# mrluin/TextualDegRemoval

Measured on AMD Instinct MI355X. Metric: train images/sec (512x512, bs=4/GPU), higher is better.
Workload: dtype f32 (3xbf16-split MFMA: 24-bit operand significands on the full fp32 exponent range, fp32 accumulate; unscaled gradients, no loss scale, no step-skip guard; tensors fp32 -- the MASA-encoder ResidualBlock activations / gradients as three bf16 planes whose sum IS the fp32 value, bit for bit)

## Files before the change

### textualdegremoval_amd/csrc/tdr_common.h

```cpp
#pragma once
#include <hip/hip_runtime.h>
#include <stdint.h>
#include <stdio.h>
#include <string.h>

#define TDR_OK 0
#define TDR_ERR_ARG (-1)
#define TDR_ERR_HIP (-2)
#define TDR_ERR_UNSUPPORTED (-3)

void tdr_set_error(const char* fmt, ...);

#define TDR_REQUIRE(cond, ...)                     \
    do {                                           \
        if (!(cond)) {                             \
            tdr_set_error(__VA_ARGS__);            \
            return TDR_ERR_ARG;                    \
        }                                          \
    } while (0)

#define TDR_LAUNCH_CHECK(name)                                                         \
    do {                                                                               \
        hipError_t e__ = hipGetLastError();                                            \
        if (e__ != hipSuccess) {                                                       \
            tdr_set_error("%s: launch failed: %s", name, hipGetErrorString(e__));      \
            return TDR_ERR_HIP;                                                        \
        }                                                                              \
    } while (0)

struct TdrConvDesc;
int tdr_conv_forward_bx3(const TdrConvDesc* d, void* stream);

static inline int tdr_cdiv(long a, long b) { return (int)((a + b - 1) / b); }

#include <stdlib.h>
#ifdef TDR_TUNING_KNOBS
static inline const char* tdr_tune_env(const char* name) { return getenv(name); }
#else
static inline const char* tdr_tune_env(const char*) { return nullptr; }
#endif

__device__ __forceinline__ int tdr_xcd_logical_block() {
    const int T = gridDim.x, b = blockIdx.x;
    const int q = T >> 3, r = T & 7, xcd = b & 7, slot = b >> 3;
    return (xcd < r ? xcd * (q + 1) : r * (q + 1) + (xcd - r) * q) + slot;
}

typedef __attribute__((ext_vector_type(16))) float f32x16;
typedef __attribute__((ext_vector_type(4))) float f32x4;

__device__ __forceinline__ float wave_sum(float v) {
#pragma unroll
    for (int o = 32; o > 0; o >>= 1) v += __shfl_xor(v, o, 64);
    return v;
}
template <int CTRL>
__device__ __forceinline__ float dpp_perm(float v) {
    return __builtin_bit_cast(float, __builtin_amdgcn_update_dpp(0, __builtin_bit_cast(int, v), CTRL, 0xf, 0xf, true));
}
__device__ __forceinline__ float wave_sum_dpp(float v) {
    v += dpp_perm<0xB1>(v);
    v += dpp_perm<0x4E>(v);
    v += dpp_perm<0x141>(v);
    v += dpp_perm<0x140>(v);
    const int b = __builtin_bit_cast(int, v);
    return (__builtin_bit_cast(float, __builtin_amdgcn_readlane(b, 0)) + __builtin_bit_cast(float, __builtin_amdgcn_readlane(b, 16))) +
           (__builtin_bit_cast(float, __builtin_amdgcn_readlane(b, 32)) + __builtin_bit_cast(float, __builtin_amdgcn_readlane(b, 48)));
}
__device__ __forceinline__ float wave_max(float v) {
#pragma unroll
    for (int o = 32; o > 0; o >>= 1) v = fmaxf(v, __shfl_xor(v, o, 64));
    return v;
}

typedef float tdr_f32x2 __attribute__((ext_vector_type(2)));
typedef _Float16 tdr_f16x2 __attribute__((ext_vector_type(2)));
template <bool PIN = true>
__device__ __forceinline__ void tdr_split2_f16(float x0, float x1, unsigned& h, unsigned& m) {
    if constexpr (PIN) asm volatile("" : "+v"(x0), "+v"(x1));
    const tdr_f32x2 xv = {x0, x1};
    h = __builtin_bit_cast(unsigned, __builtin_convertvector(xv, tdr_f16x2));
    const float neg1 = -1.0f;
    asm("v_fma_mixlo_f16 %0, %1, %2, %3 op_sel:[0,0,0] op_sel_hi:[1,0,0]" : "=v"(m) : "v"(h), "v"(neg1), "v"(x0));
    asm("v_fma_mixhi_f16 %0, %1, %2, %3 op_sel:[1,0,0] op_sel_hi:[1,0,0]" : "+v"(m) : "v"(h), "v"(neg1), "v"(x1));
}

typedef __bf16 tdr_bf16x2 __attribute__((ext_vector_type(2)));
template <bool PIN = true>
__device__ __forceinline__ void tdr_split3_bf16(float x0, float x1, unsigned& h, unsigned& m, unsigned& l) {
    if constexpr (PIN) asm volatile("" : "+v"(x0), "+v"(x1));
    const tdr_f32x2 xv = {x0, x1};
    h = __builtin_bit_cast(unsigned, __builtin_convertvector(xv, tdr_bf16x2));
    const float r0 = x0 - __builtin_bit_cast(float, h << 16), r1 = x1 - __builtin_bit_cast(float, h & 0xffff0000u);
    const tdr_f32x2 rv = {r0, r1};
    m = __builtin_bit_cast(unsigned, __builtin_convertvector(rv, tdr_bf16x2));
    const tdr_f32x2 sv = {r0 - __builtin_bit_cast(float, m << 16), r1 - __builtin_bit_cast(float, m & 0xffff0000u)};
    l = __builtin_bit_cast(unsigned, __builtin_convertvector(sv, tdr_bf16x2));
}
```

### textualdegremoval_amd/csrc/tdr_dwsg.hip

```cpp
#include <stdlib.h>
#include "tdr_common.h"
#include "tdr_erf.h"
#include "tdr_dw_stencil.h"
#include "../../include/tdr.h"

namespace {

enum { MODE_FWD = 0, MODE_DU = 1, MODE_DT = 2 };
enum { GATE_MUL = 0, GATE_GELU = 1, GATE_NONE = 2, GATE_SUM = 3 };

__device__ __forceinline__ float gelu_erf(float x) { return 0.5f * x * (1.0f + erf_1ulp(x * 0.70710678118654752f)); }
__device__ __forceinline__ void gelu_erf_both(float x, float& g, float& dg) {
    const float h = 0.5f * (1.0f + erf_1ulp(x * 0.70710678118654752f));
    g = x * h;
    dg = h + x * 0.3989422804014327f * __expf(-0.5f * x * x);
}

struct DwArgs {
    const float* a;
    const float* dg;
    const float* w;
    const float* b;
    float* out;
    float* part;
// ... 272 lines not shown
                for (int kx = 0; kx < 3; ++kx)
#pragma unroll
                    for (int e = 0; e < 4; ++e) {
                        o1[e] += w1[ky * 3 + kx] * t1[ky].v[e + kx];
                        o2[e] += w2[ky * 3 + kx] * t2[ky].v[e + kx];
                    }
            if (GATE == GATE_MUL && in_img) gv += dgb;
            float d1[4], d2[4];
#pragma unroll
            for (int e = 0; e < 4; ++e) {
                if (GATE == GATE_GELU) {
                    float gl, gd;
                    gelu_erf_both(o1[e], gl, gd);
                    d1[e] = gv[e] * o2[e] * gd;
                    d2[e] = gv[e] * gl;
                } else {
                    d1[e] = gv[e] * o2[e];
                    d2[e] = gv[e] * o1[e];
                }
                if (!in_img) { d1[e] = 0.f; d2[e] = 0.f; }
            }
            float l1 = __shfl_up(d1[3], 1, 64), r1 = __shfl_down(d1[0], 1, 64);
            float l2 = __shfl_up(d2[3], 1, 64), r2 = __shfl_down(d2[0], 1, 64);
            if (!left_lane) { l1 = 0.f; l2 = 0.f; }
            if (!right_lane) { r1 = 0.f; r2 = 0.f; }
            if (TPRW > 64) {
                const int wv = tid >> 6, par = i & 1;
                if (lane == 0) { edge[par][wv][0] = d1[0]; edge[par][wv][1] = d2[0]; }
                if (lane == 63) { edge[par][wv][2] = d1[3]; edge[par][wv][3] = d2[3]; }
                __syncthreads();
                if (lane == 0 && cg != 0) { l1 = edge[par][wv - 1][2]; l2 = edge[par][wv - 1][3]; }
                if (lane == 63 && cg != TPRW - 1) { r1 = edge[par][wv + 1][0]; r2 = edge[par][wv + 1][1]; }
            }
            e1[2].v[0] = l1; e1[2].v[5] = r1; e2[2].v[0] = l2; e2[2].v[5] = r2;
#pragma unroll
            for (int e = 0; e < 4; ++e) { e1[2].v[e + 1] = d1[e]; e2[2].v[e + 1] = d2[e]; }
        }
        if (i >= 1 && i <= a.rpt && in_img) {
#pragma unroll
            for (int ky = 0; ky < 3; ++ky)
#pragma unroll
                for (int kx = 0; kx < 3; ++kx)
#pragma unroll
                    for (int e = 0; e < 4; ++e) {
                        acc[ky * 3 + kx] += e1[2].v[e + 1] * t1[ky].v[e + kx];
                        acc[10 + ky * 3 + kx] += e2[2].v[e + 1] * t2[ky].v[e + kx];
                    }
            acc[9] += (e1[2].v[1] + e1[2].v[2]) + (e1[2].v[3] + e1[2].v[4]);
            acc[19] += (e2[2].v[1] + e2[2].v[2]) + (e2[2].v[3] + e2[2].v[4]);
        }
        if (i >= 2) {
            const int yo = y - 1;
            float o1[4] = {0.f, 0.f, 0.f, 0.f}, o2[4] = {0.f, 0.f, 0.f, 0.f};
#pragma unroll
            for (int ky = 0; ky < 3; ++ky)
#pragma unroll
                for (int kx = 0; kx < 3; ++kx)
#pragma unroll
                    for (int e = 0; e < 4; ++e) {
                        o1[e] += w1[8 - (ky * 3 + kx)] * e1[ky].v[e + kx];
                        o2[e] += w2[8 - (ky * 3 + kx)] * e2[ky].v[e + kx];
                    }
            if (active && yo < H) {
                const f32x4 v1 = {o1[0], o1[1], o1[2], o1[3]}, v2 = {o2[0], o2[1], o2[2], o2[3]};
                *reinterpret_cast<f32x4*>(a.out + ((long)n * 2 * C + pl1) * HW + (long)yo * W + x0) = v1;
                *reinterpret_cast<f32x4*>(a.out + ((long)n * 2 * C + pl2) * HW + (long)yo * W + x0) = v2;
            }
        }
        t1[0] = t1[1]; t1[1] = t1[2];
        t2[0] = t2[1]; t2[1] = t2[2];
        e1[0] = e1[1]; e1[1] = e1[2];
        e2[0] = e2[1]; e2[1] = e2[2];
    }
#pragma unroll
    for (int i = 0; i < 20; ++i) {
        const float s = wave_sum(acc[i]);
        if (lane == 0) red[tid >> 6][i] = s;
    }
    __syncthreads();
    if (tid < 20)
        a.part[(((long)n * C + c) * gridDim.x + blockIdx.x) * 20 + tid] = (red[0][tid] + red[1][tid]) + (red[2][tid] + red[3][tid]);
}

__global__ void dw_param_finish_kernel(const float* __restrict__ part, int N, int C, int nb, float* __restrict__ dw,
                                       float* __restrict__ db, int sum_pairs) {
    const int c = blockIdx.x, tid = threadIdx.x;
    if (tid >= 20) return;
    float sacc = 0.f;
    for (int m = 0; m < N; ++m)
        for (int g = 0; g < nb; ++g) sacc += part[(((long)m * C + c) * nb + g) * 20 + tid];
    const int kk = tid % 10;
    if (sum_pairs) {
        if (kk < 9) dw[(2 * c + (tid >= 10)) * 9 + kk] = sacc;
        else if (db && tid == 9) db[c] = sacc;
        return;
    }
    const int ch = tid < 10 ? c : c + C;
    if (kk < 9) dw[ch * 9 + kk] = sacc;
    else if (db) db[ch] = sacc;
}

__global__ void dw_param_finish_multi_kernel(const long long* __restrict__ tab) {
    const long long* row = tab + 6L * blockIdx.y;
    const int N = (int)row[3], C = (int)row[4], nb = (int)row[5];
    if ((int)blockIdx.x >= C) return;
    const float* part = reinterpret_cast<const float*>(row[0]);
    float* dw = reinterpret_cast<float*>(row[1]);
    float* db = reinterpret_cast<float*>(row[2]);
    const int c = blockIdx.x, tid = threadIdx.x;
    if (tid >= 20) return;
    float sacc = 0.f;
    for (int m = 0; m < N; ++m)
        for (int g = 0; g < nb; ++g) sacc += part[(((long)m * C + c) * nb + g) * 20 + tid];
    const int kk = tid % 10;
    const int ch = tid < 10 ? c : c + C;
    if (kk < 9) dw[ch * 9 + kk] = sacc;
    else db[ch] = sacc;
}

DwGeom dw_geom_fused(int H, int W) {
    DwGeom g = dw_geom(H, W);
    const int spb = 256 >> g.tprw_log2;
    static const int cap = tdr_tune_env("TDR_DWF_RPT") ? atoi(tdr_tune_env("TDR_DWF_RPT")) : 16;
    int rpt = tdr_cdiv(H, spb);
    if (rpt > cap) rpt = cap;
    if (rpt < 1) rpt = 1;
    g.rpt = rpt;
    g.nby = tdr_cdiv(H, spb * rpt);
    g.nb = g.ncb * g.nby;
    return g;
}

bool dw_two_pass() {
    const char* e = getenv("TDR_DWSG_TWO_PASS");
    return e && e[0] == '1';
}

template <int GATE>
int dw_bwd_fused(const float* t, const float* dg, const float* dg_bias, float dg_bias_mul, const float* w, const float* b, int N,
                 int C, int H, int W, float* dt, float* dw, float* db, float* ws, hipStream_t st, const float* act = nullptr,
                 long dg_ns = 0, long act_ns = 0, const float* dgB = nullptr, const float* actB = nullptr) {
    const DwGeom q = dw_geom_fused(H, W);
    DwArgs a{t, dg, w, b, dt, ws, C, H, W, q.tprw_log2, q.rpt, q.ncb, 1.0f, nullptr, nullptr, dg_bias, dg_bias_mul, act,
             {0, dg_ns, act_ns}, nullptr, 0, dgB, dg_ns, actB, act_ns};
    hipLaunchKernelGGL((dwsg_bwd_fused_kernel<GATE>), dim3(q.nb, C, N), dim3(256), 0, st, a);
    if (dw)
        hipLaunchKernelGGL(dw_param_finish_kernel, dim3(C), dim3(32), 0, st, ws, N, C, q.nb, dw, db, GATE == GATE_SUM ? 1 : 0);
    return 0;
}

}

extern "C" int64_t tdr_dwsg_ws_floats(int N, int C, int H, int W) {
    const DwGeom g = dw_geom(H, W);
    return (int64_t)N * C * g.nb * 20 + 4 + (int64_t)N * 2 * C * H * W;
}

extern "C" int tdr_dwsg_fwd(const float* t, const float* w, const float* b, int N, int C, int H, int W, float* g, float* pooled,
                            float* ws, void* stream) {
    TDR_REQUIRE(t && w && b && g && pooled && ws, "tdr_dwsg_fwd: null pointer");
    TDR_REQUIRE(W % 4 == 0, "tdr_dwsg_fwd: W must be a multiple of 4 (got %d)", W);
    hipStream_t st = (hipStream_t)stream;
    const DwGeom q = dw_geom(H, W);
    const float inv_hw = 1.0f / (float)((long)H * W);
    if (q.nb == 1) {
        DwArgs a{t, nullptr, w, b, g, pooled, C, H, W, q.tprw_log2, q.rpt, q.ncb, inv_hw};
        hipLaunchKernelGGL((dwsg_stencil_kernel<MODE_FWD, GATE_MUL>), dim3(q.nb, C, N), dim3(256), 0, st, a);
        TDR_LAUNCH_CHECK("dwsg_fwd");
        return TDR_OK;
    }
    DwArgs a{t, nullptr, w, b, g, ws, C, H, W, q.tprw_log2, q.rpt, q.ncb, 1.0f};
    hipLaunchKernelGGL((dwsg_stencil_kernel<MODE_FWD, GATE_MUL>), dim3(q.nb, C, N), dim3(256), 0, st, a);
    hipLaunchKernelGGL(dw_pool_finish_kernel, dim3(tdr_cdiv(N * C, 256)), dim3(256), 0, st, ws, N * C, q.nb, inv_hw, pooled);
    TDR_LAUNCH_CHECK("dwsg_fwd");
    return TDR_OK;
}

extern "C" int tdr_dwsg_bwd_parts_supported(int W) { return (W <= 1024 && !dw_two_pass()) ? 1 : 0; }

extern "C" int tdr_dw_param_finish(const float* ws, int N, int C, int H, int W, float* dw, float* db, void* stream) {
    TDR_REQUIRE(ws && dw && db && N > 0 && C > 0, "tdr_dw_param_finish: bad argument");
    const DwGeom q = dw_geom_fused(H, W);
    hipLaunchKernelGGL(dw_param_finish_kernel, dim3(C), dim3(32), 0, (hipStream_t)stream, const_cast<float*>(ws), N, C, q.nb, dw, db, 0);
    TDR_LAUNCH_CHECK("dw_param_finish_kernel");
    return TDR_OK;
}

extern "C" int tdr_dw_param_finish_nb(int H, int W) { return dw_geom_fused(H, W).nb; }

extern "C" int tdr_dw_param_finish_multi(const void* table, int nprob, int max_C, void* stream) {
    TDR_REQUIRE(table && nprob > 0 && max_C > 0, "tdr_dw_param_finish_multi: bad argument");
    hipLaunchKernelGGL(dw_param_finish_multi_kernel, dim3(max_C, nprob), dim3(32), 0, (hipStream_t)stream, static_cast<const long long*>(table));
    TDR_LAUNCH_CHECK("dw_param_finish_multi_kernel");
    return TDR_OK;
}

extern "C" int tdr_dwsg_bwd(const float* dg, const float* t, const float* w, const float* b, int N, int C, int H, int W,
                            float* dt, float* dw, float* db, float* ws, void* stream) {
    return tdr_dwsg_bwd_biased(dg, nullptr, 0.f, t, w, b, N, C, H, W, dt, dw, db, ws, stream);
}

extern "C" int tdr_dwsg_bwd_biased(const float* dg, const float* dg_bias, float dg_bias_mul, const float* t, const float* w,
                                   const float* b, int N, int C, int H, int W, float* dt, float* dw, float* db, float* ws,
                                   void* stream) {
    TDR_REQUIRE(dg && t && w && b && dt && ws, "tdr_dwsg_bwd: null pointer");
    TDR_REQUIRE((dw != nullptr) == (db != nullptr), "tdr_dwsg_bwd: dw and db are given together or not at all");
    TDR_REQUIRE(dw || tdr_dwsg_bwd_parts_supported(W), "tdr_dwsg_bwd: dw = db = NULL (partials left to the caller) needs the one-pass backward");
    TDR_REQUIRE(W % 4 == 0, "tdr_dwsg_bwd: W must be a multiple of 4 (got %d)", W);
    hipStream_t st = (hipStream_t)stream;
    if (W <= 1024 && !dw_two_pass()) {
        dw_bwd_fused<GATE_MUL>(t, dg, dg_bias, dg_bias_mul, w, b, N, C, H, W, dt, dw, db, ws, st);
        TDR_LAUNCH_CHECK("dwsg_bwd_fused");
        return TDR_OK;
    }
    const DwGeom q = dw_geom(H, W);
    float* part = ws;
    float* du = ws + (int64_t)N * C * q.nb * 20;
    du += (4 - (reinterpret_cast<uintptr_t>(du) / 4) % 4) % 4;
    DwArgs a1{t, dg, w, b, du, part, C, H, W, q.tprw_log2, q.rpt, q.ncb, 1.0f, nullptr, nullptr, dg_bias, dg_bias_mul};
    hipLaunchKernelGGL((dwsg_stencil_kernel<MODE_DU, GATE_MUL>), dim3(q.nb, C, N), dim3(256), 0, st, a1);
    DwArgs a2{du, nullptr, w, b, dt, part, C, H, W, q.tprw_log2, q.rpt, q.ncb, 1.0f, dw, db};
    hipLaunchKernelGGL((dwsg_stencil_kernel<MODE_DT, GATE_MUL>), dim3(q.nb, C, N), dim3(256), 0, st, a2);
    TDR_LAUNCH_CHECK("dwsg_bwd");
    return TDR_OK;
}

extern "C" int tdr_dwgelu_fwd(const float* t, const float* w, const float* b, int N, int C, int H, int W, float* g,
                              void* stream) {
// ... 127 lines not shown
```

### textualdegremoval_amd/csrc/tdr_pointwise.hip

```cpp
#include "tdr_common.h"
#include "../../include/tdr.h"

namespace {

template <int SLICES, int CPT>
__global__ __launch_bounds__(64 * SLICES) void ln_fwd_kernel(const float* __restrict__ x, long x_ns,
                                                            const float* __restrict__ w, const float* __restrict__ b,
                                                            float eps, int center, int C, int HW,
                                                            float* __restrict__ y, float* __restrict__ mu,
                                                            float* __restrict__ rstd) {
    __shared__ float red[SLICES][64];
    const int lane = threadIdx.x & 63, slice = threadIdx.x >> 6;
    const int px = blockIdx.x * 64 + lane, n = blockIdx.y;
    const bool pok = px < HW;
    const float* xn = x + (long)n * x_ns + (pok ? px : HW - 1);
    float v[CPT];
    float s = 0.f;
#pragma unroll
    for (int i = 0; i < CPT; ++i) v[i] = xn[(long)min(slice + SLICES * i, C - 1) * HW];
#pragma unroll
    for (int i = 0; i < CPT; ++i) {
        v[i] = (pok && slice + SLICES * i < C) ? v[i] : 0.f;
        s += v[i];
    }
// ... 120 lines not shown
    for (int c = slice; c < C; c += 16) yn[(long)c * HW] = (xn[(long)c * HW] - mo) * rs * w[c] + (b ? b[c] : 0.f);
    if (slice == 0) {
        mu[(long)n * HW + px] = mean;
        rstd[(long)n * HW + px] = rs;
    }
}

template <int SLICES, int CPT>
__global__ __launch_bounds__(64 * SLICES) void ln_bwd_kernel(
    const float* __restrict__ go, const float* __restrict__ x, long x_ns, const float* __restrict__ mu,
    const float* __restrict__ rstd, const float* __restrict__ w, const float* __restrict__ add, long add_ns, int add_C,
    int center, int N, int C, int HW, float* __restrict__ gx, float* __restrict__ part ) {
    __shared__ float red[2][SLICES][64];
    const int lane = threadIdx.x & 63, slice = __builtin_amdgcn_readfirstlane(threadIdx.x >> 6);
    const int tiles = (HW + 63) / 64;
    float aw[CPT], ab[CPT];
#pragma unroll
    for (int i = 0; i < CPT; ++i) { aw[i] = 0.f; ab[i] = 0.f; }
    const unsigned uHW = (unsigned)HW;
    for (int t = blockIdx.x; t < N * tiles; t += gridDim.x) {
        const int n = t / tiles, px = (t % tiles) * 64 + lane;
        const bool pok = px < HW;
        const unsigned pxc = pok ? px : HW - 1;
        const float m = mu[(long)n * HW + pxc], rs = pok ? rstd[(long)n * HW + pxc] : 0.f;
        const float* xb = x + (long)n * x_ns;
        const float* gb_ = go + (long)n * C * HW;
        float* ob = gx + (long)n * C * HW;
        float xv[CPT], g0[CPT];
#pragma unroll
        for (int i = 0; i < CPT; ++i) {
            const unsigned c = min(slice + SLICES * i, C - 1);
            xv[i] = xb[c * uHW + pxc];
            g0[i] = gb_[c * uHW + pxc];
        }
        const float off = center ? 0.f : m * rs;
        float s1 = 0.f, s2 = 0.f;
#pragma unroll
        for (int i = 0; i < CPT; ++i) {
            const int c = slice + SLICES * i;
            const bool ok = pok && c < C;
            const float gg = ok ? g0[i] : 0.f;
            const float yh = ok ? (xv[i] - m) * rs : 0.f;
            const float yu = ok ? yh + off : 0.f;
            const float gv = gg * w[min(c, C - 1)];
            xv[i] = yh; g0[i] = gv;
            s1 += gv;
            s2 += gv * yu;
            aw[i] += gg * yu;
            ab[i] += gg;
        }
        red[0][slice][lane] = s1;
        red[1][slice][lane] = s2;
        __syncthreads();
        float S1 = 0.f, S2 = 0.f;
#pragma unroll
        for (int k = 0; k < SLICES; ++k) { S1 += red[0][k][lane]; S2 += red[1][k][lane]; }
        __syncthreads();
        const float mg = center ? S1 / (float)C : 0.f, mgy = S2 / (float)C;
        float av[CPT];
        if (add) {
            const float* ab_ = add + (long)n * add_ns;
#pragma unroll
            for (int i = 0; i < CPT; ++i) av[i] = ab_[(unsigned)min(slice + SLICES * i, add_C - 1) * uHW + pxc];
        }
#pragma unroll
        for (int i = 0; i < CPT; ++i) {
            const int c = slice + SLICES * i;
            float v = rs * (g0[i] - xv[i] * mgy - mg);
            if (add && c < add_C) v += av[i];
            if (pok && c < C) ob[(unsigned)c * uHW + pxc] = v;
        }
    }
#pragma unroll
    for (int i = 0; i < CPT; ++i) {
        const int c = slice + SLICES * i;
        const float sw = wave_sum(aw[i]), sb = wave_sum(ab[i]);
        if (lane == 0 && c < C) {
            part[((long)blockIdx.x * 2 + 0) * C + c] = sw;
            part[((long)blockIdx.x * 2 + 1) * C + c] = sb;
        }
    }
}

template <bool PART>
__global__ __launch_bounds__(1024) void ln_bwd_generic_kernel(
    const float* __restrict__ go, const float* __restrict__ x, long x_ns, const float* __restrict__ mu,
    const float* __restrict__ rstd, const float* __restrict__ w, const float* __restrict__ add, long add_ns, int add_C,
    int center, int C, int HW, float* __restrict__ gx, float* __restrict__ part) {
    __shared__ float red[2][16][64];
    const int lane = threadIdx.x & 63, slice = threadIdx.x >> 6;
    const int px = blockIdx.x * 64 + lane, n = blockIdx.y;
    const bool pok = px < HW;
    const unsigned pxc = pok ? px : HW - 1, uHW = (unsigned)HW;
    const float m = mu[(long)n * HW + pxc], rs = rstd[(long)n * HW + pxc];
    const float* xb = x + (long)n * x_ns;
    const float* gb_ = go + (long)n * C * HW;
    const float off = center ? 0.f : m * rs;
    float s1 = 0.f, s2 = 0.f;
#pragma unroll 4
    for (int c = slice; c < C; c += 16) {
        const float g = gb_[(unsigned)c * uHW + pxc] * w[c];
        const float yh = (xb[(unsigned)c * uHW + pxc] - m) * rs;
        s1 += g; s2 += g * (yh + off);
    }
    red[0][slice][lane] = s1; red[1][slice][lane] = s2;
    __syncthreads();
    float S1 = 0.f, S2 = 0.f;
#pragma unroll
    for (int k = 0; k < 16; ++k) { S1 += red[0][k][lane]; S2 += red[1][k][lane]; }
    const float mg = center ? S1 / (float)C : 0.f, mgy = S2 / (float)C;
    const float* ab_ = add ? add + (long)n * add_ns : xb;
    float* ob = gx + (long)n * C * HW;
    for (int c0 = slice; c0 < C; c0 += 64) {
        float g0[4], xv[4], av[4];
#pragma unroll
        for (int k = 0; k < 4; ++k) {
            const int c = min(c0 + 16 * k, C - 1);
            g0[k] = gb_[(unsigned)c * uHW + pxc];
            xv[k] = xb[(unsigned)c * uHW + pxc];
            av[k] = ab_[(unsigned)min(c, add ? add_C - 1 : C - 1) * uHW + pxc];
        }
#pragma unroll
        for (int k = 0; k < 4; ++k) {
            const int c = c0 + 16 * k;
            if (c < C) {
                const float g = g0[k] * w[c];
                const float yh = (xv[k] - m) * rs;
                float v = rs * (g - yh * mgy - mg);
                if (add && c < add_C) v += av[k];
                if (pok) ob[(unsigned)c * uHW + pxc] = v;
                if (PART) {
                    const float sw = wave_sum(pok ? g0[k] * (yh + off) : 0.f), sb = wave_sum(pok ? g0[k] : 0.f);
                    if (lane == 0) {
                        float* pb = part + ((long)(blockIdx.y * gridDim.x + blockIdx.x) * 2) * C;
                        pb[c] = sw;
                        pb[C + c] = sb;
                    }
                }
            }
        }
    }
}

template <int CPT>
__global__ __launch_bounds__(1024) void ln_bwd_cached_kernel(
    const float* __restrict__ go, const float* __restrict__ x, long x_ns, const float* __restrict__ mu,
    const float* __restrict__ rstd, const float* __restrict__ w, const float* __restrict__ add, long add_ns, int add_C,
    int center, int C, int HW, float* __restrict__ gx, float* __restrict__ part) {
    __shared__ float red[2][16][64];
    const int lane = threadIdx.x & 63, slice = __builtin_amdgcn_readfirstlane(threadIdx.x >> 6);
    const int px = blockIdx.x * 64 + lane, n = blockIdx.y;
    const bool pok = px < HW;
    const unsigned pxc = pok ? px : HW - 1;
    const float* xb = x + (long)n * x_ns;
    const float* gb_ = go + (long)n * C * HW;
    float g0[CPT], xv[CPT];
#pragma unroll
    for (int i = 0; i < CPT; ++i) {
        const long row = (long)min(slice + 16 * i, C - 1) * HW;
        g0[i] = (gb_ + row)[pxc];
        xv[i] = (xb + row)[pxc];
    }
    const float m = mu[(long)n * HW + pxc], rs = rstd[(long)n * HW + pxc];
    const float off = center ? 0.f : m * rs;
    float s1 = 0.f, s2 = 0.f;
#pragma unroll
    for (int i = 0; i < CPT; ++i) {
        const int c = slice + 16 * i;
        const float wc = c < C ? w[min(c, C - 1)] : 0.f;
        g0[i] = c < C ? g0[i] : 0.f;
        xv[i] = (xv[i] - m) * rs;
        const float g = g0[i] * wc;
        s1 += g; s2 += g * (xv[i] + off);
    }
    red[0][slice][lane] = s1; red[1][slice][lane] = s2;
    __syncthreads();
    float S1 = 0.f, S2 = 0.f;
#pragma unroll
    for (int k = 0; k < 16; ++k) { S1 += red[0][k][lane]; S2 += red[1][k][lane]; }
    const float mg = center ? S1 / (float)C : 0.f, mgy = S2 / (float)C;
    const float* ab_ = add ? add + (long)n * add_ns : xb;
    float* ob = gx + (long)n * C * HW;
    float* pb = part + ((long)(blockIdx.y * gridDim.x + blockIdx.x) * 2) * C;
#pragma unroll
    for (int i = 0; i < CPT; ++i) {
        const int c = slice + 16 * i, cc = min(c, C - 1);
        const long row = (long)cc * HW;
        float v = rs * (g0[i] * w[cc] - xv[i] * mgy - mg);
        const float av = (ab_ + (long)min(cc, add ? add_C - 1 : C - 1) * HW)[pxc];
        if (add && c < add_C) v += av;
        const float sw = wave_sum_dpp(pok ? g0[i] * (xv[i] + off) : 0.f), sb = wave_sum_dpp(pok ? g0[i] : 0.f);
        if (c < C) {
            if (pok) (ob + row)[pxc] = v;
            if (lane == 0) { pb[c] = sw; pb[C + c] = sb; }
        }
    }
}

__global__ __launch_bounds__(256) void ln_param_grad_kernel(const float* __restrict__ go, const float* __restrict__ x,
                                                           long x_ns, const float* __restrict__ mu,
                                                           const float* __restrict__ rstd, int center, int N, int C,
                                                           int HW, float* __restrict__ part) {
    __shared__ float red[2][4];
    const int c = blockIdx.x, split = blockIdx.y, nsplit = gridDim.y;
    const long total = (long)N * HW;
    float sw = 0.f, sb = 0.f;
    for (long i = (long)split * 256 + threadIdx.x; i < total; i += (long)nsplit * 256) {
        const int n = (int)(i / HW), px = (int)(i % HW);
        const float g0 = go[((long)n * C + c) * HW + px];
        const float yh = (x[(long)n * x_ns + (long)c * HW + px] - (center ? mu[i] : 0.f)) * rstd[i];
        sw += g0 * yh; sb += g0;
    }
    sw = wave_sum(sw); sb = wave_sum(sb);
    if ((threadIdx.x & 63) == 0) { red[0][threadIdx.x >> 6] = sw; red[1][threadIdx.x >> 6] = sb; }
    __syncthreads();
    if (threadIdx.x == 0) {
        part[((long)split * 2 + 0) * C + c] = red[0][0] + red[0][1] + red[0][2] + red[0][3];
        part[((long)split * 2 + 1) * C + c] = red[1][0] + red[1][1] + red[1][2] + red[1][3];
    }
}

template <int KL>
__global__ __launch_bounds__(64 * KL) void pair_sum_partials_kernel(const float* __restrict__ part, int nparts, int C,
                                                                    float* __restrict__ o0, float* __restrict__ o1) {
    __shared__ float red[KL][64];
    const int lane = threadIdx.x & 63, kl = threadIdx.x >> 6;
    const int e = blockIdx.x * 64 + lane;
    const int ec = e < C ? e : C - 1;
    const float* p = part + (long)blockIdx.y * C + ec;
    const long stride = 2L * C;
    float s0 = 0.f, s1 = 0.f;
    int k = kl;
    for (; k + KL < nparts; k += 2 * KL) { s0 += p[(long)k * stride]; s1 += p[(long)(k + KL) * stride]; }
    if (k < nparts) s0 += p[(long)k * stride];
    red[kl][lane] = s0 + s1;
    __syncthreads();
    if (kl == 0 && e < C) {
        float t = 0.f;
#pragma unroll
        for (int q = 0; q < KL; ++q) t += red[q][lane];
        (blockIdx.y ? o1 : o0)[e] = t;
    }
}

template <int KL>
__global__ __launch_bounds__(64 * KL) void pair_sum_partials_multi_kernel(const long long* __restrict__ tab) {
    __shared__ float red[KL][64];
    const long long* row = tab + 5L * blockIdx.z;
    const int nparts = (int)row[3], C = (int)row[4];
    if ((int)blockIdx.x * 64 >= C) return;
    const float* part = reinterpret_cast<const float*>(row[0]);
    float* o = reinterpret_cast<float*>(blockIdx.y ? row[2] : row[1]);
    const int lane = threadIdx.x & 63, kl = threadIdx.x >> 6;
    const int e = blockIdx.x * 64 + lane;
    const int ec = e < C ? e : C - 1;
    const float* p = part + (long)blockIdx.y * C + ec;
    const long stride = 2L * C;
    float s0 = 0.f, s1 = 0.f;
    int k = kl;
    for (; k + KL < nparts; k += 2 * KL) { s0 += p[(long)k * stride]; s1 += p[(long)(k + KL) * stride]; }
    if (k < nparts) s0 += p[(long)k * stride];
    red[kl][lane] = s0 + s1;
    __syncthreads();
    if (kl == 0 && e < C) {
        float t = 0.f;
#pragma unroll
        for (int q = 0; q < KL; ++q) t += red[q][lane];
        o[e] = t;
    }
}

constexpr int LN_BWD_GRID = 1024;
static const int ln_bwd_grid = tdr_tune_env("TDR_LN_BWD_GRID") ? atoi(tdr_tune_env("TDR_LN_BWD_GRID")) : 256;
constexpr int LN_GEN_SPLITS = 16;

__global__ __launch_bounds__(256) void sca_fwd_kernel(const float* __restrict__ pooled, const float* __restrict__ wsca,
                                                     const float* __restrict__ bsca, int C, float* __restrict__ s) {
    const int co = blockIdx.x * 4 + (threadIdx.x >> 6), n = blockIdx.y, lane = threadIdx.x & 63;
    if (co >= C) return;
    float a = 0.f;
    for (int ci = lane; ci < C; ci += 64) a += wsca[(long)co * C + ci] * pooled[(long)n * C + ci];
    a = wave_sum(a);
    if (lane == 0) s[(long)n * C + co] = a + bsca[co];
}

__global__ __launch_bounds__(256) void sca_bwd_rows_kernel(const float* __restrict__ G3, const float* __restrict__ S3,
                                                          const float* __restrict__ w3, const float* __restrict__ b3,
                                                          const float* __restrict__ beta, const float* __restrict__ s,
                                                          int N, int C, float* __restrict__ dw3, float* __restrict__ db3,
                                                          float* __restrict__ dbeta) {
    __shared__ float red[4];
    const int co = blockIdx.x;
    const float bt = beta[co];
    float acc = 0.f;
    for (int ci = threadIdx.x; ci < C; ci += 256) {
        float sg = 0.f;
        for (int n = 0; n < N; ++n) sg += s[(long)n * C + ci] * G3[((long)n * C + co) * C + ci];
        dw3[(long)co * C + ci] = bt * sg;
        acc += w3[(long)co * C + ci] * sg;
    }
    acc = wave_sum(acc);
    if ((threadIdx.x & 63) == 0) red[threadIdx.x >> 6] = acc;
    __syncthreads();
    if (threadIdx.x == 0) {
        const float tot = (red[0] + red[1]) + (red[2] + red[3]);
        db3[co] = bt * S3[co];
        dbeta[co] = tot + b3[co] * S3[co];
    }
}

__global__ __launch_bounds__(1024) void sca_bwd_ds_kernel(const float* __restrict__ G3, const float* __restrict__ w3,
                                                         const float* __restrict__ beta, int N, int C, float* __restrict__ ds) {
    __shared__ float red[16][64];
    const int lane = threadIdx.x & 63, sl = threadIdx.x >> 6;
    const int ci = blockIdx.x * 64 + lane, n = blockIdx.y;
    const int cic = min(ci, C - 1);
    float a = 0.f;
    for (int co = sl; co < C; co += 16) a += beta[co] * w3[(long)co * C + cic] * G3[((long)n * C + co) * C + cic];
    red[sl][lane] = a;
    __syncthreads();
    if (sl == 0 && ci < C) {
        float t = 0.f;
#pragma unroll
        for (int q = 0; q < 16; ++q) t += red[q][lane];
        ds[(long)n * C + ci] = t;
    }
}

__global__ void sca_bwd_dw_kernel(const float* __restrict__ ds, const float* __restrict__ pooled, int N, int C,
                                  float* __restrict__ dwsca) {
    const int cj = blockIdx.x * blockDim.x + threadIdx.x, ci = blockIdx.y;
    if (cj >= C) return;
    float a = 0.f;
    for (int n = 0; n < N; ++n) a += ds[(long)n * C + ci] * pooled[(long)n * C + cj];
    dwsca[(long)ci * C + cj] = a;
}

__global__ __launch_bounds__(1024) void sca_bwd_tail_kernel(const float* __restrict__ ds, const float* __restrict__ wsca,
                                                           int N, int C, float* __restrict__ dbsca,
                                                           float* __restrict__ dpooled) {
    __shared__ float red[16][64];
    const int lane = threadIdx.x & 63, sl = threadIdx.x >> 6;
    const int cj = blockIdx.x * 64 + lane, n = blockIdx.y;
    const int cjc = min(cj, C - 1);
    float a = 0.f;
    for (int ci = sl; ci < C; ci += 16) a += wsca[(long)ci * C + cjc] * ds[(long)n * C + ci];
    red[sl][lane] = a;
    __syncthreads();
    if (sl == 0 && cj < C) {
        float t = 0.f;
#pragma unroll
        for (int q = 0; q < 16; ++q) t += red[q][lane];
        dpooled[(long)n * C + cj] = t;
        if (n == 0) {
            float sb = 0.f;
            for (int m = 0; m < N; ++m) sb += ds[(long)m * C + cj];
            dbsca[cj] = sb;
// ... 288 lines not shown
    for (int k = 0; k < PSNR_BLOCKS; ++k) s += part[n * PSNR_BLOCKS + k];
    return s / (double)cnt;
}
__global__ __launch_bounds__(256) void psnr_grad_kernel(const float* __restrict__ p, const float* __restrict__ t, long CHW, long HW,
                                                       int toY, int N, float wscale, const TdrStepGuard* __restrict__ guard,
                                                       const double* __restrict__ part, float* __restrict__ dpred) {
    const int n = blockIdx.y;
    const long base = (long)n * CHW, cnt = toY ? HW : CHW;
    float gscale = wscale;
    if (guard) gscale *= guard->scale;
    const float f = (float)((double)gscale / (double)N / (psnr_image_mse(part, n, cnt) + 1e-8) * 2.0 / (double)cnt);
    for (long i = blockIdx.x * 256L + threadIdx.x; i < cnt; i += (long)gridDim.x * 256) {
        const float d = psnr_diff(p, t, base, HW, i, toY);
        if (!toY) {
            dpred[base + i] = f * d;
        } else {
            dpred[base + i] = f * d * (65.481f / 255.f);
            dpred[base + HW + i] = f * d * (128.553f / 255.f);
            dpred[base + 2 * HW + i] = f * d * (24.966f / 255.f);
        }
    }
}
__global__ void psnr_finish_kernel(const double* __restrict__ part, int N, long cnt, double wscale, float* __restrict__ loss) {
    double s = 0.0;
    for (int n = threadIdx.x; n < N; n += 64) s += log(psnr_image_mse(part, n, cnt) + 1e-8);
#pragma unroll
    for (int o = 32; o > 0; o >>= 1) s += __shfl_xor(s, o, 64);
    if (threadIdx.x == 0) loss[0] = (float)(s / (double)N * wscale);
}

inline int grid1d(long total, int cap = 8192) {
    long b = (total + 255) / 256;
    return (int)(b < cap ? (b < 1 ? 1 : b) : cap);
}

}

extern "C" int tdr_layernorm2d_fwd(const float* x, int64_t x_ns, const float* w, const float* b, float eps, int center,
                                   int N, int C, int HW, float* y, float* mu, float* rstd, void* stream) {
    TDR_REQUIRE(x && w && y && mu && rstd, "tdr_layernorm2d_fwd: null pointer");
    TDR_REQUIRE(N > 0 && C > 0 && HW > 0, "tdr_layernorm2d_fwd: bad shape");
    hipStream_t st = (hipStream_t)stream;
    dim3 grid(tdr_cdiv(HW, 64), N);
#define LN_FWD(S, P) hipLaunchKernelGGL((ln_fwd_kernel<S, P>), grid, dim3(64 * S), 0, st, x, (long)x_ns, w, b, eps, center, C, HW, y, mu, rstd)
    if (C <= 32) LN_FWD(4, 8);
    else if (C <= 64) LN_FWD(4, 16);
    else if (C <= 128) LN_FWD(4, 32);
    else if (C <= 256) LN_FWD(8, 32);
    else if (C <= 512) LN_FWD(16, 32);
    else if (C <= 64 * 24 && (long)grid.x * N < 512) {
        dim3 g16(tdr_cdiv(HW, 16), N);
        if (C <= 64 * 12) hipLaunchKernelGGL(ln_fwd_narrow_kernel<12>, g16, dim3(1024), 0, st, x, (long)x_ns, w, b, eps, center, C, HW, y, mu, rstd);
        else hipLaunchKernelGGL(ln_fwd_narrow_kernel<24>, g16, dim3(1024), 0, st, x, (long)x_ns, w, b, eps, center, C, HW, y, mu, rstd);
    }
    else hipLaunchKernelGGL(ln_fwd_generic_kernel, grid, dim3(1024), 0, st, x, (long)x_ns, w, b, eps, center, C, HW, y, mu, rstd);
#undef LN_FWD
    TDR_LAUNCH_CHECK("ln_fwd");
    return TDR_OK;
}

extern "C" int64_t tdr_ln_ws_floats(int N, int C, int HW) {
    (void)N; (void)HW;
    return (int64_t)LN_BWD_GRID * 2 * C;
}

extern "C" int tdr_layernorm2d_bwd(const float* go, const float* x, int64_t x_ns, const float* mu, const float* rstd,
                                   const float* w, const float* add, int64_t add_ns, int add_C, int center, int N, int C,
                                   int HW, float* gx, float* gw, float* gb, float* ws, void* stream) {
    TDR_REQUIRE(go && x && mu && rstd && w && gx && gw && gb && ws, "tdr_layernorm2d_bwd: null pointer");
    hipStream_t st = (hipStream_t)stream;
    const int tiles = tdr_cdiv(HW, 64) * N;
    int nparts;
    if (C <= 128) {
        const int cap = ln_bwd_grid < 1 ? 1 : (ln_bwd_grid > LN_BWD_GRID ? LN_BWD_GRID : ln_bwd_grid);
        const int grid = tiles < cap ? tiles : cap;
        nparts = grid;
#define LN_BWD(S, P) hipLaunchKernelGGL((ln_bwd_kernel<S, P>), dim3(grid), dim3(64 * S), 0, st, go, x, (long)x_ns, mu, rstd, w, add, (long)add_ns, add_C, center, N, C, HW, gx, ws)
        if (C <= 32) LN_BWD(4, 8);
        else if (C <= 64) LN_BWD(4, 16);
        else LN_BWD(8, 16);
#undef LN_BWD
    } else {
        static const bool fuse = tdr_tune_env("TDR_LN_NOFUSE") == nullptr;
        if (tiles <= LN_BWD_GRID && fuse) {
            static const bool cached = tdr_tune_env("TDR_LN_NOCACHE") == nullptr;
#define LN_BWDC(P) hipLaunchKernelGGL(ln_bwd_cached_kernel<P>, dim3(tdr_cdiv(HW, 64), N), dim3(1024), 0, st, go, x, (long)x_ns, mu, rstd, w, add, (long)add_ns, add_C, center, C, HW, gx, ws)
            if (cached && C <= 256) LN_BWDC(16);
            else if (cached && C <= 512) LN_BWDC(32);
            else
                hipLaunchKernelGGL(ln_bwd_generic_kernel<true>, dim3(tdr_cdiv(HW, 64), N), dim3(1024), 0, st, go, x, (long)x_ns,
                                   mu, rstd, w, add, (long)add_ns, add_C, center, C, HW, gx, ws);
#undef LN_BWDC
            nparts = tiles;
        } else {
            hipLaunchKernelGGL(ln_bwd_generic_kernel<false>, dim3(tdr_cdiv(HW, 64), N), dim3(1024), 0, st, go, x, (long)x_ns, mu,
                               rstd, w, add, (long)add_ns, add_C, center, C, HW, gx, (float*)nullptr);
            hipLaunchKernelGGL(ln_param_grad_kernel, dim3(C, LN_GEN_SPLITS), dim3(256), 0, st, go, x, (long)x_ns, mu, rstd, center,
                               N, C, HW, ws);
            nparts = LN_GEN_SPLITS;
        }
    }
    hipLaunchKernelGGL(pair_sum_partials_kernel<16>, dim3(tdr_cdiv(C, 64), 2), dim3(1024), 0, st, ws, nparts, C, gw, gb);
    TDR_LAUNCH_CHECK("ln_bwd");
    return TDR_OK;
}

__global__ __launch_bounds__(256) void pair_fold_partials_kernel(const float* __restrict__ part, int nparts, int C2,
                                                                float* __restrict__ mid) {
    __shared__ float red[256];
    const int SL = C2 >= 256 ? 1 : 256 / C2;
    const int el = SL > 1 ? (int)threadIdx.x % C2 : (int)threadIdx.x, sl = SL > 1 ? (int)threadIdx.x / C2 : 0;
    const int e = SL > 1 ? el : blockIdx.x * 256 + el;
    const bool live = e < C2 && sl < SL;
    const int per = 256 / SL;
    const int r0 = blockIdx.y * 256 + sl * per, r1 = min(r0 + per, nparts);
    float s0 = 0.f, s1 = 0.f, s2 = 0.f, s3 = 0.f;
    if (live) {
        int r = r0;
        for (; r + 3 < r1; r += 4) {
            s0 += part[(long)r * C2 + e]; s1 += part[(long)(r + 1) * C2 + e];
            s2 += part[(long)(r + 2) * C2 + e]; s3 += part[(long)(r + 3) * C2 + e];
        }
        for (; r < r1; ++r) s0 += part[(long)r * C2 + e];
    }
    const float t = (s0 + s1) + (s2 + s3);
    if (SL == 1) {
        if (live) mid[(long)blockIdx.y * C2 + e] = t;
        return;
    }
    red[threadIdx.x] = live ? t : 0.f;
    __syncthreads();
    if (sl == 0 && e < C2) {
        float a = 0.f;
        for (int q = 0; q < SL; ++q) a += red[q * C2 + el];
        mid[(long)blockIdx.y * C2 + e] = a;
    }
}

extern "C" int64_t tdr_pair_sum_mid_floats(int nparts, int C) { return nparts > 1024 ? (int64_t)tdr_cdiv(nparts, 256) * 2 * C : 0; }

extern "C" int tdr_pair_sum_partials(const float* part, int nparts, int C, float* o0, float* o1, float* mid, void* stream) {
    TDR_REQUIRE(part && o0 && o1 && nparts > 0 && C > 0, "tdr_pair_sum_partials: bad argument");
    hipStream_t st = (hipStream_t)stream;
    if (nparts > 1024) {
        TDR_REQUIRE(mid, "tdr_pair_sum_partials: %d partial rows need the fold scratch", nparts);
        const int S = tdr_cdiv(nparts, 256);
        hipLaunchKernelGGL(pair_fold_partials_kernel, dim3(tdr_cdiv(2 * C, 256), S), dim3(256), 0, st, part, nparts, 2 * C, mid);
        part = mid;
        nparts = S;
    }
    hipLaunchKernelGGL(pair_sum_partials_kernel<16>, dim3(tdr_cdiv(C, 64), 2), dim3(1024), 0, st, part, nparts, C, o0, o1);
    TDR_LAUNCH_CHECK("pair_sum_partials");
    return TDR_OK;
}

extern "C" int tdr_pair_sum_partials_multi(const void* table, int nprob, int max_C, void* stream) {
    TDR_REQUIRE(table && nprob > 0 && max_C > 0, "tdr_pair_sum_partials_multi: bad argument");
    hipLaunchKernelGGL(pair_sum_partials_multi_kernel<16>, dim3(tdr_cdiv(max_C, 64), 2, nprob), dim3(1024), 0, (hipStream_t)stream,
                       static_cast<const long long*>(table));
    TDR_LAUNCH_CHECK("pair_sum_partials_multi");
    return TDR_OK;
}

extern "C" int tdr_scaled_conv_param_grads_multi(const void* table, int nprob, int max_Cout, void* stream) {
    TDR_REQUIRE(table && nprob > 0 && max_Cout > 0, "tdr_scaled_conv_param_grads_multi: bad argument");
    hipLaunchKernelGGL(scaled_conv_param_multi_kernel, dim3(max_Cout, nprob), dim3(256), 0, (hipStream_t)stream, static_cast<const long long*>(table));
    TDR_LAUNCH_CHECK("scaled_conv_param_multi_kernel");
    return TDR_OK;
// ... 213 lines not shown
```

Before: 62.24.

## Add multi-plane-per-block dwsg backward and 16-pixel LN backward tiles for small maps

```diff
diff --git a/profiles/small_maps/compare_dumps.py b/profiles/small_maps/compare_dumps.py
--- /dev/null
+++ b/profiles/small_maps/compare_dumps.py
@@ -0,0 +1,21 @@
+import itertools
+import os
+import sys
+
+import numpy as np
+
+
+def main():
+    dirs = [a.split('=', 1) for a in sys.argv[1:]]
+    for (na, da), (nb, db) in itertools.combinations(dirs, 2):
+        print(f'{na} vs {nb}')
+        for f in sorted(os.listdir(da)):
+            if not f.endswith('.npy') or not os.path.exists(os.path.join(db, f)):
+                continue
+            a, b = np.load(os.path.join(da, f)), np.load(os.path.join(db, f))
+            d = float(np.abs(a.astype(np.float64) - b.astype(np.float64)).max())
+            print(f'{f} {a.shape} {"identical" if d == 0 else "DIFFERENT"} max|d|={d:.3e}')
+
+
+if __name__ == '__main__':
+    main()
diff --git a/profiles/small_maps/kernel_times.py b/profiles/small_maps/kernel_times.py
--- /dev/null
+++ b/profiles/small_maps/kernel_times.py
@@ -0,0 +1,38 @@
+import re
+import sqlite3
+import statistics
+import sys
+
+
+def main():
+    db = sys.argv[1]
+    pat = re.compile(sys.argv[2] if len(sys.argv) > 2 else r'dwsg_bwd_fused|ln_bwd_|ln_fwd_')
+    skip = int(sys.argv[3]) if len(sys.argv) > 3 else 0
+    runs = len(sys.argv) > 4 and sys.argv[4] == 'runs'
+    rows, last, seg = {}, None, 0
+    q = 'select name, grid_x/workgroup_x, grid_y, grid_z, workgroup_x, end-start, vgpr_count, lds_size from kernels order by start'
+    for name, gx, gy, gz, wg, dur, vg, lds in sqlite3.connect(db).execute(q):
+        if pat.search(name):
+            n = re.sub(r'\(anonymous namespace\)::|^void |\(.*', '', name)
+            key = (n, gx, gy, gz, wg, vg, lds)
+            if runs and key != last:
+                seg += 1
+            last = key
+            rows.setdefault((seg,) + key, []).append(dur / 1e3)
+    print(f'{"n":>5} {"min us":>8} {"median":>8} {"mean":>8}  kernel, grid (workgroups x,y,z), threads, vgpr column, lds')
+    steps = int(sys.argv[4][6:]) if len(sys.argv) > 4 and sys.argv[4].startswith('steps=') else 0
+    table = []
+    for (seg, n, gx, gy, gz, wg, vg, lds), d in rows.items():
+        m = len(d) // steps if steps and len(d) % steps == 0 else 1
+        label = f'{n} grid({gx},{gy},{gz}) x{wg} vgpr {vg} lds {lds}'
+        if 1 < m <= 4:
+            table += [(seg, f'{label}  launch {p + 1} of {m} in the step', d[p::m]) for p in range(m)]
+        else:
+            table.append((seg, label, d))
+    for seg, label, d in sorted(table, key=lambda r: (r[0], r[1])):
+        d = d[skip:] if len(d) > skip else d
+        print(f'{len(d):5d} {min(d):8.1f} {statistics.median(d):8.1f} {statistics.mean(d):8.1f}  {label}')
+
+
+if __name__ == '__main__':
+    main()
diff --git a/profiles/small_maps/probe_small_maps.py b/profiles/small_maps/probe_small_maps.py
--- /dev/null
+++ b/profiles/small_maps/probe_small_maps.py
@@ -0,0 +1,58 @@
+import os
+import sys
+
+import torch
+
+sys.path.insert(0, os.path.join(os.path.dirname(os.path.abspath(__file__)), os.pardir, os.pardir))
+from textualdegremoval_amd import kernels as K
+
+SETS, REPS = 5, 30
+DW_SHAPES = [(4, 256, 64, 64), (4, 512, 64, 64), (4, 512, 32, 32), (4, 1024, 32, 32)]
+LN_SHAPES = [(4, 1024, 32, 32), (4, 512, 32, 32), (4, 256, 64, 64)]
+
+
+def dw(forms):
+    for N, C, H, W in DW_SHAPES:
+        sets = [(torch.randn(N, C, H, W, device='cuda'), torch.randn(N, 2 * C, H, W, device='cuda')) for _ in range(SETS)]
+        w = torch.randn(2 * C, 1, 3, 3, device='cuda') * 0.4
+        b = torch.randn(2 * C, device='cuda') * 0.2
+        for form in forms:
+            if form is None:
+                os.environ.pop('TDR_DWSG_PLANE', None)
+            else:
+                os.environ['TDR_DWSG_PLANE'] = form
+            for i in range(REPS):
+                dg, t = sets[i % SETS]
+                K.dwsg_bwd(dg, t, w, b, defer_finish=True)
+            torch.cuda.synchronize()
+        os.environ.pop('TDR_DWSG_PLANE', None)
+        del sets
+
+
+def ln(forms):
+    for N, C, H, W in LN_SHAPES:
+        sets = []
+        wt = torch.randn(C, device='cuda') * 0.3 + 1
+        bs = torch.randn(C, device='cuda') * 0.2
+        for _ in range(SETS):
+            x = torch.randn(N, C, H, W, device='cuda')
+            _, mu, rs = K.layernorm2d_fwd(x, wt, bs, 1e-6)
+            sets.append((torch.randn(N, C, H, W, device='cuda'), x, mu, rs, torch.randn(N, C, H, W, device='cuda')))
+        for form in forms:
+            if form is None:
+                os.environ.pop('TDR_LN_TILE16', None)
+            else:
+                os.environ['TDR_LN_TILE16'] = form
+            for i in range(REPS):
+                go, x, mu, rs, add = sets[i % SETS]
+                K.layernorm2d_bwd(go, x, mu, rs, wt, add=add)
+            torch.cuda.synchronize()
+        os.environ.pop('TDR_LN_TILE16', None)
+        del sets
+
+
+if __name__ == '__main__':
+    dw_forms = ['0', None] + (['2', '4'] if '--tuning' in sys.argv else [])
+    dw(dw_forms)
+    ln(['0', None])
+    print('probe_small_maps: done')
diff --git a/textualdegremoval_amd/csrc/tdr_common.h b/textualdegremoval_amd/csrc/tdr_common.h
--- a/textualdegremoval_amd/csrc/tdr_common.h
+++ b/textualdegremoval_amd/csrc/tdr_common.h
@@ -32,6 +32,15 @@
 int tdr_conv_forward_bx3(const TdrConvDesc* d, void* stream);
 
 static inline int tdr_cdiv(long a, long b) { return (int)((a + b - 1) / b); }
+
+static inline int tdr_cu_count() {
+    static const int cus = [] {
+        int dev = 0, n = 0;
+        if (hipGetDevice(&dev) != hipSuccess || hipDeviceGetAttribute(&n, hipDeviceAttributeMultiprocessorCount, dev) != hipSuccess) n = 0;
+        return n;
+    }();
+    return cus;
+}
 
 #include <stdlib.h>
 #ifdef TDR_TUNING_KNOBS
diff --git a/textualdegremoval_amd/csrc/tdr_dwsg.hip b/textualdegremoval_amd/csrc/tdr_dwsg.hip
--- a/textualdegremoval_amd/csrc/tdr_dwsg.hip
+++ b/textualdegremoval_amd/csrc/tdr_dwsg.hip
@@ -378,6 +378,147 @@
         a.part[(((long)n * C + c) * gridDim.x + blockIdx.x) * 20 + tid] = (red[0][tid] + red[1][tid]) + (red[2][tid] + red[3][tid]);
 }
 
+template <int PPW>
+__global__ __launch_bounds__(256) void dwsg_bwd_small_kernel(DwArgs a) {
+    __shared__ float red[4][20];
+    constexpr int TPP = 256 / PPW;
+    const int tid = threadIdx.x, lane = tid & 63;
+    const int n = blockIdx.z, C = a.C, H = a.H, W = a.W;
+    const int cw = __builtin_amdgcn_readfirstlane(blockIdx.y * PPW + tid / TPP);
+    const int c = min(cw, C - 1);
+    const int TPRW = 1 << a.tprw_log2;
+    const int cg = tid & (TPRW - 1), strip = (tid & (TPP - 1)) >> a.tprw_log2;
+    const int x0 = cg * 4;
+    const int ybeg = strip * a.rpt;
+    const bool active = x0 < W && ybeg < H && cw < C;
+    const bool left_lane = lane != 0 && cg != 0;
+    const bool right_lane = lane != 63 && cg != TPRW - 1;
+    const long HW = (long)H * W;
+    const float* p1 = a.a + ((long)n * 2 * C + c) * HW;
+    const float* p2 = a.a + ((long)n * 2 * C + c + C) * HW;
+    const float* q1 = a.dg + ((long)n * C + c) * HW;
+    float w1[9], w2[9];
+#pragma unroll
+    for (int i = 0; i < 9; ++i) {
+        w1[i] = a.w[c * 9 + i];
+        w2[i] = a.w[(c + C) * 9 + i];
+    }
+    const float b1 = a.b[c], b2 = a.b[c + C];
+    const float dgb = a.dgb ? a.dgb[(long)n * C + c] * a.dgb_mul : 0.f;
+    float acc[20];
+#pragma unroll
+    for (int i = 0; i < 20; ++i) acc[i] = 0.f;
+
+    Row6 t1[3], t2[3], e1[3], e2[3];
+#pragma unroll
+    for (int k = 0; k < 6; ++k) { e1[0].v[k] = e1[1].v[k] = e2[0].v[k] = e2[1].v[k] = 0.f; }
+    t1[0] = fetch_row(p1, ybeg - 2, x0, H, W, active, left_lane, right_lane);
+    t2[0] = fetch_row(p2, ybeg - 2, x0, H, W, active, left_lane, right_lane);
+    t1[1] = fetch_row(p1, ybeg - 1, x0, H, W, active, left_lane, right_lane);
+    t2[1] = fetch_row(p2, ybeg - 1, x0, H, W, active, left_lane, right_lane);
+    auto dg_row = [&](int y, bool on) {
+        f32x4 g = {0.f, 0.f, 0.f, 0.f};
+        if (on && y >= 0 && y < H) g = *reinterpret_cast<const f32x4*>(q1 + (long)y * W + x0);
+        return g;
+    };
+    constexpr int AHEAD = 1;
+    RawRow n1[AHEAD], n2[AHEAD];
+    f32x4 gn[AHEAD];
+#pragma unroll
+    for (int k = 0; k < AHEAD; ++k) {
+        n1[k] = load_raw(p1, ybeg + k, x0, H, W, active, left_lane, right_lane);
+        n2[k] = load_raw(p2, ybeg + k, x0, H, W, active, left_lane, right_lane);
+        gn[k] = dg_row(ybeg - 1 + k, active);
+    }
+    const int iters = a.rpt + 2;
+    for (int i0 = 0; i0 < iters; i0 += AHEAD) {
+#pragma unroll
+        for (int k = 0; k < AHEAD; ++k) {
+            const int i = i0 + k;
+            if (i >= iters) break;
+            const int y = ybeg - 1 + i;
+            f32x4 gv = gn[k];
+            t1[2] = finish_row(n1[k], left_lane, right_lane);
+            t2[2] = finish_row(n2[k], left_lane, right_lane);
+            const bool more = active && i + AHEAD < iters;
+            n1[k] = load_raw(p1, y + 1 + AHEAD, x0, H, W, more, left_lane, right_lane);
+            n2[k] = load_raw(p2, y + 1 + AHEAD, x0, H, W, more, left_lane, right_lane);
+            gn[k] = dg_row(y + AHEAD, more);
+            const bool in_img = active && y >= 0 && y < H;
+            float o1[4] = {b1, b1, b1, b1}, o2[4] = {b2, b2, b2, b2};
+#pragma unroll
+            for (int ky = 0; ky < 3; ++ky)
+#pragma unroll
+                for (int kx = 0; kx < 3; ++kx)
+#pragma unroll
+                    for (int e = 0; e < 4; ++e) {
+                        o1[e] += w1[ky * 3 + kx] * t1[ky].v[e + kx];
+                        o2[e] += w2[ky * 3 + kx] * t2[ky].v[e + kx];
+                    }
+            if (in_img) gv += dgb;
+            float d1[4], d2[4];
+#pragma unroll
+            for (int e = 0; e < 4; ++e) {
+                d1[e] = gv[e] * o2[e];
+                d2[e] = gv[e] * o1[e];
+                if (!in_img) { d1[e] = 0.f; d2[e] = 0.f; }
+            }
+            float l1 = __shfl_up(d1[3], 1, 64), r1 = __shfl_down(d1[0], 1, 64);
+            float l2 = __shfl_up(d2[3], 1, 64), r2 = __shfl_down(d2[0], 1, 64);
+            if (!left_lane) { l1 = 0.f; l2 = 0.f; }
+            if (!right_lane) { r1 = 0.f; r2 = 0.f; }
+            e1[2].v[0] = l1; e1[2].v[5] = r1; e2[2].v[0] = l2; e2[2].v[5] = r2;
+#pragma unroll
+            for (int e = 0; e < 4; ++e) { e1[2].v[e + 1] = d1[e]; e2[2].v[e + 1] = d2[e]; }
+            if (i >= 1 && i <= a.rpt && in_img) {
+#pragma unroll
+                for (int ky = 0; ky < 3; ++ky)
+#pragma unroll
+                    for (int kx = 0; kx < 3; ++kx)
+#pragma unroll
+                        for (int e = 0; e < 4; ++e) {
+                            acc[ky * 3 + kx] += e1[2].v[e + 1] * t1[ky].v[e + kx];
+                            acc[10 + ky * 3 + kx] += e2[2].v[e + 1] * t2[ky].v[e + kx];
+                        }
+                acc[9] += (e1[2].v[1] + e1[2].v[2]) + (e1[2].v[3] + e1[2].v[4]);
+                acc[19] += (e2[2].v[1] + e2[2].v[2]) + (e2[2].v[3] + e2[2].v[4]);
+            }
+            if (i >= 2) {
+                const int yo = y - 1;
+                float u1[4] = {0.f, 0.f, 0.f, 0.f}, u2[4] = {0.f, 0.f, 0.f, 0.f};
+#pragma unroll
+                for (int ky = 0; ky < 3; ++ky)
+#pragma unroll
+                    for (int kx = 0; kx < 3; ++kx)
+#pragma unroll
+                        for (int e = 0; e < 4; ++e) {
+                            u1[e] += w1[8 - (ky * 3 + kx)] * e1[ky].v[e + kx];
+                            u2[e] += w2[8 - (ky * 3 + kx)] * e2[ky].v[e + kx];
+                        }
+                if (active && yo < H) {
+                    const f32x4 v1 = {u1[0], u1[1], u1[2], u1[3]}, v2 = {u2[0], u2[1], u2[2], u2[3]};
+                    *reinterpret_cast<f32x4*>(a.out + ((long)n * 2 * C + c) * HW + (long)yo * W + x0) = v1;
+                    *reinterpret_cast<f32x4*>(a.out + ((long)n * 2 * C + c + C) * HW + (long)yo * W + x0) = v2;
+                }
+            }
+            t1[0] = t1[1]; t1[1] = t1[2];
+            t2[0] = t2[1]; t2[1] = t2[2];
+            e1[0] = e1[1]; e1[1] = e1[2];
+            e2[0] = e2[1]; e2[1] = e2[2];
+        }
+    }
+#pragma unroll
+    for (int i = 0; i < 20; ++i) {
+        const float s = wave_sum(acc[i]);
+        if (lane == 0) red[tid >> 6][i] = s;
+    }
+    __syncthreads();
+    if (tid < 20 * PPW) {
+        const int s = tid / 20, i = tid % 20, cs = blockIdx.y * PPW + s;
+        if (cs < C) a.part[((long)n * C + cs) * 20 + i] = PPW == 2 ? red[2 * s][i] + red[2 * s + 1][i] : red[s][i];
+    }
+}
+
 __global__ void dw_param_finish_kernel(const float* __restrict__ part, int N, int C, int nb, float* __restrict__ dw,
                                        float* __restrict__ db, int sum_pairs) {
     const int c = blockIdx.x, tid = threadIdx.x;
@@ -414,9 +555,9 @@
     else db[ch] = sacc;
 }
 
-DwGeom dw_geom_fused(int H, int W) {
+DwGeom dw_geom_fused(int H, int W, int ppw = 1) {
     DwGeom g = dw_geom(H, W);
-    const int spb = 256 >> g.tprw_log2;
+    const int spb = (256 / ppw) >> g.tprw_log2;
     static const int cap = tdr_tune_env("TDR_DWF_RPT") ? atoi(tdr_tune_env("TDR_DWF_RPT")) : 16;
     int rpt = tdr_cdiv(H, spb);
     if (rpt > cap) rpt = cap;
@@ -427,6 +568,16 @@
     return g;
 }
 
+int dw_small_ppw(int N, int C, int H, int W) {
+    if (H > 64 || W > 64) return 1;
+    const char* e = getenv("TDR_DWSG_PLANE");
+    if (e && e[0] == '0') return 1;
+#ifdef TDR_TUNING_KNOBS
+    if (e && (e[0] == '2' || e[0] == '4')) return e[0] - '0';
+#endif
+    return (W <= 32 || tdr_cdiv((long)N * C, 2) > 3 * tdr_cu_count()) ? 4 : 2;
+}
+
 bool dw_two_pass() {
     const char* e = getenv("TDR_DWSG_TWO_PASS");
     return e && e[0] == '1';
@@ -436,10 +587,13 @@
 int dw_bwd_fused(const float* t, const float* dg, const float* dg_bias, float dg_bias_mul, const float* w, const float* b, int N,
                  int C, int H, int W, float* dt, float* dw, float* db, float* ws, hipStream_t st, const float* act = nullptr,
                  long dg_ns = 0, long act_ns = 0, const float* dgB = nullptr, const float* actB = nullptr) {
-    const DwGeom q = dw_geom_fused(H, W);
+    const int ppw = GATE == GATE_MUL ? dw_small_ppw(N, C, H, W) : 1;
+    const DwGeom q = dw_geom_fused(H, W, ppw);
     DwArgs a{t, dg, w, b, dt, ws, C, H, W, q.tprw_log2, q.rpt, q.ncb, 1.0f, nullptr, nullptr, dg_bias, dg_bias_mul, act,
              {0, dg_ns, act_ns}, nullptr, 0, dgB, dg_ns, actB, act_ns};
-    hipLaunchKernelGGL((dwsg_bwd_fused_kernel<GATE>), dim3(q.nb, C, N), dim3(256), 0, st, a);
+    if (ppw == 2) hipLaunchKernelGGL(dwsg_bwd_small_kernel<2>, dim3(1, tdr_cdiv(C, 2), N), dim3(256), 0, st, a);
+    else if (ppw == 4) hipLaunchKernelGGL(dwsg_bwd_small_kernel<4>, dim3(1, tdr_cdiv(C, 4), N), dim3(256), 0, st, a);
+    else hipLaunchKernelGGL((dwsg_bwd_fused_kernel<GATE>), dim3(q.nb, C, N), dim3(256), 0, st, a);
     if (dw)
         hipLaunchKernelGGL(dw_param_finish_kernel, dim3(C), dim3(32), 0, st, ws, N, C, q.nb, dw, db, GATE == GATE_SUM ? 1 : 0);
     return 0;
diff --git a/textualdegremoval_amd/csrc/tdr_pointwise.hip b/textualdegremoval_amd/csrc/tdr_pointwise.hip
--- a/textualdegremoval_amd/csrc/tdr_pointwise.hip
+++ b/textualdegremoval_amd/csrc/tdr_pointwise.hip
@@ -226,14 +226,22 @@
     }
 }
 
-template <bool PART>
-__global__ __launch_bounds__(1024) void ln_bwd_generic_kernel(
+template <int PXT>
+__device__ __forceinline__ float ln_tile_sum(float v) {
+    if (PXT == 64) return wave_sum(v);
+#pragma unroll
+    for (int o = 8; o > 0; o >>= 1) v += __shfl_xor(v, o, 64);
+    return v;
+}
+
+template <bool PART, int PXT = 64>
+__global__ __launch_bounds__(16 * PXT) void ln_bwd_generic_kernel(
     const float* __restrict__ go, const float* __restrict__ x, long x_ns, const float* __restrict__ mu,
     const float* __restrict__ rstd, const float* __restrict__ w, const float* __restrict__ add, long add_ns, int add_C,
     int center, int C, int HW, float* __restrict__ gx, float* __restrict__ part) {
-    __shared__ float red[2][16][64];
-    const int lane = threadIdx.x & 63, slice = threadIdx.x >> 6;
-    const int px = blockIdx.x * 64 + lane, n = blockIdx.y;
+    __shared__ float red[2][16][PXT];
+    const int lane = threadIdx.x & (PXT - 1), slice = threadIdx.x / PXT;
+    const int px = blockIdx.x * PXT + lane, n = blockIdx.y;
     const bool pok = px < HW;
     const unsigned pxc = pok ? px : HW - 1, uHW = (unsigned)HW;
     const float m = mu[(long)n * HW + pxc], rs = rstd[(long)n * HW + pxc];
@@ -274,7 +282,7 @@
                 if (add && c < add_C) v += av[k];
                 if (pok) ob[(unsigned)c * uHW + pxc] = v;
                 if (PART) {
-                    const float sw = wave_sum(pok ? g0[k] * (yh + off) : 0.f), sb = wave_sum(pok ? g0[k] : 0.f);
+                    const float sw = ln_tile_sum<PXT>(pok ? g0[k] * (yh + off) : 0.f), sb = ln_tile_sum<PXT>(pok ? g0[k] : 0.f);
                     if (lane == 0) {
                         float* pb = part + ((long)(blockIdx.y * gridDim.x + blockIdx.x) * 2) * C;
                         pb[c] = sw;
@@ -417,6 +425,11 @@
 constexpr int LN_BWD_GRID = 1024;
 static const int ln_bwd_grid = tdr_tune_env("TDR_LN_BWD_GRID") ? atoi(tdr_tune_env("TDR_LN_BWD_GRID")) : 256;
 constexpr int LN_GEN_SPLITS = 16;
+
+bool ln_tile16_on() {
+    const char* e = getenv("TDR_LN_TILE16");
+    return !(e && e[0] == '0');
+}
 
 __global__ __launch_bounds__(256) void sca_fwd_kernel(const float* __restrict__ pooled, const float* __restrict__ wsca,
                                                      const float* __restrict__ bsca, int C, float* __restrict__ s) {
@@ -871,8 +884,13 @@
 #undef LN_BWD
     } else {
         static const bool fuse = tdr_tune_env("TDR_LN_NOFUSE") == nullptr;
-        if (tiles <= LN_BWD_GRID && fuse) {
-            static const bool cached = tdr_tune_env("TDR_LN_NOCACHE") == nullptr;
+        static const bool cached = tdr_tune_env("TDR_LN_NOCACHE") == nullptr;
+        const int tiles16 = tdr_cdiv(HW, 16) * N;
+        if ((C > 512 || !cached) && tiles < tdr_cu_count() && tiles16 <= LN_BWD_GRID && fuse && ln_tile16_on()) {
+            hipLaunchKernelGGL((ln_bwd_generic_kernel<true, 16>), dim3(tdr_cdiv(HW, 16), N), dim3(256), 0, st, go, x, (long)x_ns, mu, rstd,
+                               w, add, (long)add_ns, add_C, center, C, HW, gx, ws);
+            nparts = tiles16;
+        } else if (tiles <= LN_BWD_GRID && fuse) {
 #define LN_BWDC(P) hipLaunchKernelGGL(ln_bwd_cached_kernel<P>, dim3(tdr_cdiv(HW, 64), N), dim3(1024), 0, st, go, x, (long)x_ns, mu, rstd, w, add, (long)add_ns, add_C, center, C, HW, gx, ws)
             if (cached && C <= 256) LN_BWDC(16);
             else if (cached && C <= 512) LN_BWDC(32);
```

Result: no change. 62.54, median of 6 (+0.5%).
